# isarandi/metrabs

Measured on AMD Instinct MI355X. Metric: crops/sec (256px, 72 depth bins) at 1/2/4/8 MI355X; MPJPE vs ref, higher is better.
Workload: dtype f32

## Files before the change

### metrabs_amd/backbones.py

```python
import collections
import threading

import torch
import torch.nn.functional as F
from torch import nn


class DepthwiseConv2d(nn.Conv2d):

    use_miopen = False
    _backend_lock = threading.Lock()

    def forward(self, x):
        if x.is_cuda and not DepthwiseConv2d.use_miopen and torch.backends.cudnn.enabled:
            cudnn = torch.backends.cudnn
            with DepthwiseConv2d._backend_lock, cudnn.flags(
                    enabled=False, benchmark=cudnn.benchmark, deterministic=cudnn.deterministic,
                    allow_tf32=cudnn.allow_tf32):
                return super().forward(x)
        return super().forward(x)


class ConvBNAct(nn.Sequential):

# ... 211 lines not shown
        self.b = ConvBNAct(cout, cout, 3, 1, act=None, eps=1e-5)
        self.down = None if stride == 1 and cin == cout else ConvBNAct(cin, cout, 1, stride, act=None, eps=1e-5)

    def forward(self, x):
        idt = x if self.down is None else self.down(x)
        return torch.relu(self.b(self.a(x)) + idt)


def resnet18():
    layers = [ConvBNAct(3, 64, 7, 2, act=nn.ReLU, eps=1e-5), nn.MaxPool2d(3, 2, 1)]
    cin = 64
    for cout, stride in [(64, 1), (128, 2), (256, 2), (512, 2)]:
        layers += [BasicBlock(cin, cout, stride), BasicBlock(cout, cout, 1)]
        cin = cout
    net = nn.Sequential(*layers)
    net.out_channels = 512
    return net


class MBv3Block(nn.Module):
    def __init__(self, cin, k, exp, cout, se, hs, stride):
        super().__init__()
        act = nn.Hardswish if hs else nn.ReLU
        self.residual = stride == 1 and cin == cout
        layers = []
        if exp != cin:
            layers.append(ConvBNAct(cin, exp, 1, 1, act=act))
        layers.append(ConvBNAct(exp, exp, k, stride, groups=exp, act=act))
        if se:
            layers.append(SqueezeExcite(exp, max(8, exp // 4), gate=nn.Hardsigmoid, act=nn.ReLU))
        layers.append(ConvBNAct(exp, cout, 1, 1, act=None))
        self.block = nn.Sequential(*layers)

    def forward(self, x):
        return _block_plus_skip(self.block, x) if self.residual else self.block(x)


def mobilenet_v3_large():
    table = [(3, 16, 16, 0, 0, 1), (3, 64, 24, 0, 0, 2), (3, 72, 24, 0, 0, 1), (5, 72, 40, 1, 0, 2),
             (5, 120, 40, 1, 0, 1), (5, 120, 40, 1, 0, 1), (3, 240, 80, 0, 1, 2), (3, 200, 80, 0, 1, 1),
             (3, 184, 80, 0, 1, 1), (3, 184, 80, 0, 1, 1), (3, 480, 112, 1, 1, 1), (3, 672, 112, 1, 1, 1),
             (5, 672, 160, 1, 1, 2), (5, 960, 160, 1, 1, 1), (5, 960, 160, 1, 1, 1)]
    layers = [Preproc(), ConvBNAct(3, 16, 3, 2, act=nn.Hardswish)]
    cin = 16
    for k, exp, cout, se, hs, s in table:
        layers.append(MBv3Block(cin, k, exp, cout, bool(se), bool(hs), s))
        cin = cout
    layers += [ConvBNAct(cin, 960, 1, 1, act=nn.Hardswish), ConvBNAct(960, 1280, 1, 1, act=nn.Hardswish)]
    net = nn.Sequential(*layers)
    net.out_channels = 1280
    return net


def build_backbone(name):
    name = name.lower()
    if name in ('efficientnetv2-s', 'effnetv2-s', 'effv2s'):
        return efficientnetv2('s')
    if name in ('efficientnetv2-l', 'effnetv2-l', 'effv2l'):
        return efficientnetv2('l')
    if name in ('resnet18', 'resnet-18'):
        return resnet18()
    if name in ('mobilenetv3', 'mobilenetv3-large', 'mobilenet-v3'):
        return mobilenet_v3_large()
    raise ValueError(f'unknown backbone {name}')


_ACT_NAMES = {nn.SiLU: 'silu', nn.ReLU: 'relu', nn.Hardswish: 'hardswish'}


class ConvBiasAct(nn.Module):

    def __init__(self, conv, bias, act):
        super().__init__()
        self.conv = conv
        self.register_buffer('bias', bias.detach().float().contiguous())
        self.act = act
        self.act_name = None if act is None else _ACT_NAMES[type(act)]
        self.emit_mean = False
        self._mean = None
        self._gate = None
        self.last_path = None

    use_k13 = True
    k13_slower = frozenset({(1536, 256, 64)})

    def k13_takes(self, x):
        c = self.conv
        if not (ConvBiasAct.use_k13 and not self.emit_mean and x.is_cuda and c.kernel_size == (1, 1)
                and c.stride == (1, 1) and c.padding == (0, 0) and c.dilation == (1, 1) and c.groups == 1
                and c.bias is None and c.padding_mode == 'zeros'):
            return False
        if torch.is_autocast_enabled('cuda') or (torch.is_grad_enabled() and c.weight.requires_grad):
            return False
        if x.dim() != 4 or (c.in_channels, c.out_channels, x.shape[2] * x.shape[3]) in ConvBiasAct.k13_slower:
            return False
        from . import kernels
        return kernels.conv1x1_supported(x, c.weight)

    def k13_accepts(self, x, residual):
        return self.k13_takes(x) and (residual is None or (residual.dtype == x.dtype and residual.is_contiguous()
                                                           and residual.data_ptr() % 16 == 0))

    use_k13h = True
    k13h_slower = frozenset({(192, 48, 4096), (256, 64, 1024), (1536, 256, 64), (256, 64, 9216), (768, 192, 576),
                             (1152, 224, 576), (1344, 224, 576), (1344, 384, 144), (2304, 384, 144),
                             (2304, 640, 144), (640, 3840, 144), (3840, 640, 144), (640, 1280, 144)})

    def k13h_takes(self, x):
        return self._k13h_takes(x, ConvBiasAct.k13h_slower)

    def _k13h_takes(self, x, slower):
        c = self.conv
        if not (ConvBiasAct.use_k13h and not self.emit_mean and x.is_cuda and x.dtype == c.weight.dtype
                and x.dtype in (torch.float16, torch.bfloat16) and c.kernel_size == (1, 1)
                and c.stride == (1, 1) and c.padding == (0, 0) and c.dilation == (1, 1) and c.groups == 1
                and c.bias is None and c.padding_mode == 'zeros'):
            return False
        if torch.is_autocast_enabled('cuda') or (torch.is_grad_enabled() and c.weight.requires_grad):
            return False
        if x.dim() != 4 or (c.in_channels, c.out_channels, x.shape[2] * x.shape[3]) in slower:
            return False
        from . import kernels
        return kernels.conv1x1_16_supported(x, c.weight)

    deep_projects = False
    deep_config = 'deepk'
    k13h_deep_slower = frozenset({(3840, 640, 144)})

    def k13h_deep_takes(self, x):
        return self.deep_projects and self._k13h_takes(x, ConvBiasAct.k13h_deep_slower)

    def give_gate(self, x, gate):
        self._gate = (x, gate)

    def take_mean_f32(self, x):
        held, self._mean = self._mean, None
        if held is not None and held[0] is x:
            return held[1]
        return None

    def take_mean(self, x):
        m = self.take_mean_f32(x)
        return None if m is None else m.to(x.dtype).view(x.shape[0], x.shape[1], 1, 1)

    def forward(self, x, residual=None, defer_epilogue=False, pre=None):
        if defer_epilogue:
            self.last_path = 'library'
            return self.conv(x)
        if pre is not None:
            from . import kernels
            self._gate, self.last_path = None, 'k13'
            return kernels.conv1x1_bias_act(x, self.conv.weight, self.bias, self.act_name, residual=residual,
                                            in_bias=pre.bias, in_act=pre.act_name)
        held, self._gate = self._gate, None
        gate = held[1] if held is not None and held[0] is x else None
        w16 = self.conv.weight.dtype
        if x.dtype != w16 and w16 in (torch.float16, torch.bfloat16) and not torch.is_autocast_enabled(x.device.type):
            x = x.to(w16)
        skip_ok = residual is None or (residual.dtype == x.dtype and residual.is_contiguous()
                                       and residual.data_ptr() % 16 == 0)
        if skip_ok and self.k13h_deep_takes(x):
            from . import kernels
            self.last_path = 'k13h_deep' if gate is None else 'k13h_deep_gate'
            return kernels.conv1x1_bias_act16(x, self.conv.weight, self.bias, self.act_name, gate=gate,
                                              residual=residual, config=ConvBiasAct.deep_config)
        if skip_ok and self.k13h_takes(x):
            from . import kernels
# ... 359 lines not shown
```

### metrabs_amd/csrc/conv1x1.hip

```cpp
#include <type_traits>

#include "common.h"

namespace mtr {

typedef float f32x16 __attribute__((ext_vector_type(16)));

constexpr int kC1PadX = 32;
constexpr int kC1PadW = 4;

template <int WM, int WN, int FM, int FN, int BK, int ACT, int PRE>
__global__ __launch_bounds__(64 * WM * WN) void conv1x1_kernel(
    const float* __restrict__ x, const float* __restrict__ w, const float* __restrict__ bias,
    const float* __restrict__ in_bias, const float* __restrict__ gate, const float* __restrict__ residual,
    float* __restrict__ y, int M, int K, int HW, int n_total, FastDiv by_hw) {
  constexpr int NT = 64 * WM * WN;
  constexpr int BM = 32 * FM * WM, BN = 32 * FN * WN;
  constexpr int LDX = BN + kC1PadX, LDW = BM + kC1PadW;
  constexpr int XROW4 = BN / 4;
  constexpr int XPASS = NT / XROW4;
  constexpr int XV = (BK + XPASS - 1) / XPASS;
  constexpr int WPASS = NT / (BK / 4);
  constexpr int WV = (BM + WPASS - 1) / WPASS;
  static_assert(NT % XROW4 == 0 && NT % (BK / 4) == 0, "loader mapping");
// ... 180 lines not shown
  auto store_tile = [&](int stage, int kt, auto set) {
    constexpr int P = decltype(set)::value;
    const int k0 = kt * kDkBK;
    const float g = has_gate ? rg[P] : 1.0f;
    const bool x_ok = xcol_ok && k0 + xk < K;
    float* xd = &xs[stage * XS + xk * kDkBN + xp];
    float v0 = rx[P][0], v1 = rx[P][XV - 1];
    if constexpr (PRE >= 0) {
      v0 = settled(activate<PRE>(v0 + rbi[P]));
      if constexpr (XV == 2) v1 = settled(activate<PRE>(v1 + rbi[P]));
    }
    if constexpr (XV == 2) {
      *reinterpret_cast<float2*>(xd) = make_float2(x_ok ? v0 * g : 0.0f, x_ok ? v1 * g : 0.0f);
    } else {
      *xd = x_ok ? v0 * g : 0.0f;
    }
    const bool k_ok = k0 + wk4 * 4 < K;
#pragma unroll
    for (int v = 0; v < 4; ++v) {
      const int row = wr0 + v * (NT / 8);
      const bool ok = k_ok && m0 + row < M;
      float4 u = rw[P][v];
      u.x = ok ? u.x : 0.0f; u.y = ok ? u.y : 0.0f; u.z = ok ? u.z : 0.0f; u.w = ok ? u.w : 0.0f;
      *reinterpret_cast<float4*>(&ws[stage * WS + row * kDkLDW + wk4 * 4]) = u;
    }
  };

  f32x4 acc[2];
#pragma unroll
  for (int f = 0; f < 2; ++f)
#pragma unroll
    for (int r = 0; r < 4; ++r) acc[f][r] = 0.0f;

  const int c = lane & 15, kg = lane >> 4;
  auto multiply = [&](int stage, int kk0) {
    const float* xb_ = &xs[stage * XS + kg * kDkBN + c];
    const float* wb_ = &ws[stage * WS + (wave * 32 + c) * kDkLDW + kg];
#pragma unroll
    for (int kk = kk0; kk < kk0 + kDkBK / 2; kk += 4) {
      const float a = xb_[kk * kDkBN];
      const float b0 = wb_[kk], b1 = wb_[16 * kDkLDW + kk];
      acc[0] = __builtin_amdgcn_mfma_f32_16x16x4f32(a, b0, acc[0], 0, 0, 0);
      acc[1] = __builtin_amdgcn_mfma_f32_16x16x4f32(a, b1, acc[1], 0, 0, 0);
    }
  };

  const int n_tiles = (K + kDkBK - 1) / kDkBK;
  constexpr std::integral_constant<int, 0> ra{};
  constexpr std::integral_constant<int, 1> rb{};
  load_tile(0, ra);
  if (n_tiles > 1) load_tile(1, rb);
  store_tile(0, 0, ra);
  if (n_tiles > 1) store_tile(1, 1, rb);
  if (n_tiles > 2) load_tile(2, ra);
  __syncthreads();
  int stage = 0;
  auto step = [&](int t, auto hold, auto issue, auto guarded) {
    constexpr bool G = decltype(guarded)::value;
    if (!G || t + 3 < n_tiles) load_tile(t + 3, issue);
    multiply(stage, 0);
    __builtin_amdgcn_sched_barrier(0);
    if (!G || t + 2 < n_tiles) store_tile(stage == 0 ? 2 : stage - 1, t + 2, hold);
    __builtin_amdgcn_sched_barrier(0);
    multiply(stage, kDkBK / 2);
    stage = stage == 2 ? 0 : stage + 1;
    __syncthreads();
  };
  int t = 0;
  for (; t + 4 < n_tiles; t += 2) {
    step(t, ra, rb, std::false_type{});
    step(t + 1, rb, ra, std::false_type{});
  }
  for (; t < n_tiles; t += 2) {
    step(t, ra, rb, std::true_type{});
    if (t + 1 < n_tiles) step(t + 1, rb, ra, std::true_type{});
  }

  const int col = n0 + 4 * kg;
  if (col >= n_total) return;
  const unsigned b = fastdiv((unsigned)col, by_hw);
#pragma unroll
  for (int f = 0; f < 2; ++f) {
    const int m = m0 + wave * 32 + f * 16 + c;
    if (m >= M) continue;
    const float bm = bias[m];
    const long long off = ((long long)b * M + m) * HW + (col - (int)b * HW);
    float4 r;
    r.x = activate<ACT>(acc[f][0] + bm);
    r.y = activate<ACT>(acc[f][1] + bm);
    r.z = activate<ACT>(acc[f][2] + bm);
    r.w = activate<ACT>(acc[f][3] + bm);
    if (residual) {
      const float4 q = *reinterpret_cast<const float4*>(residual + off);
      r.x += q.x; r.y += q.y; r.z += q.z; r.w += q.w;
    }
    *reinterpret_cast<float4*>(y + off) = r;
  }
}

constexpr int kStR = 16;
constexpr int kStWaves = 4;
constexpr size_t kStMaxWeight = 64 * 1024;

inline int stream_kpad(int K) { return (K + 2 * kStR - 1) / (2 * kStR) * (2 * kStR); }
inline bool stream_fits(int M, int K) {
  return M <= 96 && (size_t)stream_kpad(K) * ((M + 31) / 32 * 32) * sizeof(float) <= kStMaxWeight;
}

template <int MT, int PRE, bool GATE>
__global__ __launch_bounds__(64 * kStWaves) void conv1x1_stream_kernel(
    const float* __restrict__ x, const float* __restrict__ w, const float* __restrict__ bias,
    const float* __restrict__ in_bias, const float* __restrict__ gate, const float* __restrict__ residual,
    float* __restrict__ y, int M, int K, int HW, int n_total, FastDiv by_hw, int act, int tiles) {
  constexpr int NT = 64 * kStWaves, LDW = 32 * MT;
  extern __shared__ float4 st_lds[];
  const int Kpad = (K + 2 * kStR - 1) / (2 * kStR) * (2 * kStR);
  float* ws = reinterpret_cast<float*>(st_lds);
  float* bs = ws + Kpad * LDW;

  const int tid = threadIdx.x, lane = tid & 63, wave = tid >> 6;
  const int half = lane >> 5, l32 = lane & 31;
  const long long khw = (long long)K * HW;
  const int n_chunks = Kpad / (2 * kStR);
  const int n0 = blockIdx.x * (32 * kStWaves * tiles);

  int col0 = 0;
  bool ok = false;
  const float* xsrc = x;
  const float* gsrc = x;
  auto enter_tile = [&](int tile) {
    col0 = n0 + tile * 32;
    const int col = col0 + l32;
    ok = col < n_total;
    const unsigned b = ok ? fastdiv((unsigned)col, by_hw) : 0u;
    xsrc = x + (long long)b * khw + (long long)half * HW + (ok ? col - (int)b * HW : 0);
    if constexpr (GATE) gsrc = gate + (long long)b * K + half;
  };

  float xa[kStR], xb[kStR], ga[kStR], gb[kStR];
  auto load_chunk = [&](int c, float (&xr)[kStR], float (&gr)[kStR]) {
#pragma unroll
    for (int j = 0; j < kStR; ++j) {
      const int kk = min(c * (2 * kStR) + 2 * j, K - 2);
      xr[j] = xsrc[(long long)kk * HW];
      if constexpr (GATE) gr[j] = gsrc[kk];
    }
  };

  f32x16 acc[MT];
  auto multiply_chunk = [&](int c, const float (&xr)[kStR], const float (&gr)[kStR]) {
#pragma unroll
    for (int j = 0; j < kStR; ++j) {
      const int k = c * (2 * kStR) + 2 * j;
      float v = xr[j];
      if constexpr (PRE >= 0) v = settled(activate<PRE>(v + bs[k + half]));
      if constexpr (GATE) v *= gr[j];
      v = (ok && k < K) ? v : 0.0f;
      const float* wb_ = &ws[(k + half) * LDW + l32];
#pragma unroll
      for (int i = 0; i < MT; ++i) acc[i] = __builtin_amdgcn_mfma_f32_32x32x2f32(v, wb_[i * 32], acc[i], 0, 0, 0);
    }
  };

  enter_tile(wave);
  load_chunk(0, xa, ga);

  for (int e = tid; e < (Kpad / 4) * LDW; e += NT) {
    const int m = e % LDW, k = (e / LDW) * 4;
    float4 t = make_float4(0.0f, 0.0f, 0.0f, 0.0f);
    if (m < M && k < K) t = *reinterpret_cast<const float4*>(w + (long long)m * K + k);
    float* d = &ws[k * LDW + m];
    d[0] = t.x; d[LDW] = t.y; d[2 * LDW] = t.z; d[3 * LDW] = t.w;
  }
  if constexpr (PRE >= 0)
    for (int k = tid; k < Kpad; k += NT) bs[k] = k < K ? in_bias[k] : 0.0f;
  __syncthreads();

  for (int tile = wave;;) {
#pragma unroll
    for (int i = 0; i < MT; ++i)
#pragma unroll
      for (int r = 0; r < 16; ++r) acc[i][r] = 0.0f;
    int c = 0;
    for (; c + 1 < n_chunks; c += 2) {
      load_chunk(c + 1, xb, gb);
      multiply_chunk(c, xa, ga);
      load_chunk(c + 2, xa, ga);
      multiply_chunk(c + 1, xb, gb);
    }
    if (c < n_chunks) multiply_chunk(c, xa, ga);

    auto epilogue = [&](auto act_c) {
      constexpr int ACT = decltype(act_c)::value;
#pragma unroll
      for (int i = 0; i < MT; ++i) {
        const int m = i * 32 + l32;
        if (m >= M) continue;
        const float bm = bias[m];
#pragma unroll
        for (int g = 0; g < 4; ++g) {
          const int col = col0 + 8 * g + 4 * half;
          if (col >= n_total) continue;
          const unsigned b = fastdiv((unsigned)col, by_hw);
          const long long off = ((long long)b * M + m) * HW + (col - (int)b * HW);
          float4 r;
          r.x = activate<ACT>(acc[i][4 * g + 0] + bm);
          r.y = activate<ACT>(acc[i][4 * g + 1] + bm);
          r.z = activate<ACT>(acc[i][4 * g + 2] + bm);
          r.w = activate<ACT>(acc[i][4 * g + 3] + bm);
          if (residual) {
            const float4 q = *reinterpret_cast<const float4*>(residual + off);
            r.x += q.x; r.y += q.y; r.z += q.z; r.w += q.w;
          }
          *reinterpret_cast<float4*>(y + off) = r;
        }
      }
    };
    switch (act) {
      case kActRelu: epilogue(std::integral_constant<int, kActRelu>{}); break;
      case kActSilu: epilogue(std::integral_constant<int, kActSilu>{}); break;
      case kActHardswish: epilogue(std::integral_constant<int, kActHardswish>{}); break;
      default: epilogue(std::integral_constant<int, kActNone>{}); break;
    }

    tile += kStWaves;
    if (tile >= kStWaves * tiles) break;
    enter_tile(tile);
    load_chunk(0, xa, ga);
  }
}

enum Conv1x1Config { kCfgWide = 0, kCfgSquare = 1, kCfgTall = 2, kCfgDeepK = 3, kCfgStream = 4, kCfgCount = 5 };

struct Conv1x1Plan { int cfg, waves_m, bm, bn; };

inline Conv1x1Plan plan_tall(int M) {
  const int w = M <= 160 ? (M + 31) / 32 : 4;
  return {kCfgTall, w, 32 * w, 32};
}
inline Conv1x1Plan plan_deepk(int M) {
  const int w = M <= 128 ? 4 : 8;
  return {kCfgDeepK, w, 32 * w, kDkBN};
}

inline Conv1x1Plan plan_stream(int M, int K, int HW, long long B) {
  if (!stream_fits(M, K)) return plan_tall(M);
  const int t = (B * HW + 127) / 128 >= 2048 ? 2 : 1;
  return {kCfgStream, (M + 31) / 32, (M + 31) / 32 * 32, 32 * kStWaves * t};
}

inline Conv1x1Plan pick_config(int M, int K, int HW, long long B) {
  const long long n_total = B * HW;
  const long long n_tiles128 = (n_total + 127) / 128;
  if (M == 48 && K <= 192 && HW == 4096 && stream_fits(M, K)) return plan_stream(M, K, HW, B);
  if (M <= 160) return plan_tall(M);
  if (M == 256 && K >= 512) return HW <= 64 ? plan_deepk(M) : plan_tall(M);
  if (M >= 1024 && M % 128 == 0 && K <= 256 && n_tiles128 <= 32) return plan_tall(M);
  if (M % 192 == 0 && (M / 192) * n_tiles128 >= 512) return {kCfgWide, 2, 192, 128};
  return {kCfgSquare, 2, 128, 128};
}

inline int plan_for(int M, int K, int HW, long long B, int config, Conv1x1Plan* p) {
  switch (config) {
    case -1: *p = pick_config(M, K, HW, B); return MTR_OK;
    case kCfgWide: *p = {kCfgWide, 2, 192, 128}; return MTR_OK;
    case kCfgSquare: *p = {kCfgSquare, 2, 128, 128}; return MTR_OK;
    case kCfgTall: *p = plan_tall(M); return MTR_OK;
    case kCfgDeepK: *p = plan_deepk(M); return MTR_OK;
    case kCfgStream: *p = plan_stream(M, K, HW, B); return MTR_OK;
    default: return MTR_E_PARAM;
  }
}

template <int WM, int WN, int FM, int FN, int BK, int PRE>
static int launch_conv1x1_pre(const float* x, const float* w, const float* bias, const float* in_bias,
                              const float* gate, const float* residual, float* y, int act, int M, int K, int HW,
                              long long n_total, hipStream_t stream) {
  constexpr int BM = 32 * FM * WM, BN = 32 * FN * WN;
  const long long gx = (n_total + BN - 1) / BN, gy = (M + BM - 1) / BM;
  if (gx > 0x7fffffffLL || gy > 65535) return MTR_E_SHAPE;
  const dim3 grid((unsigned)gx, (unsigned)gy), block(64 * WM * WN);
  const FastDiv by_hw = make_fastdiv((unsigned)HW);
  MTR_CLEAR_STALE();
#define MTR_C1_LAUNCH(ACT)                                                                                      \
  hipLaunchKernelGGL((conv1x1_kernel<WM, WN, FM, FN, BK, ACT, PRE>), grid, block, 0, stream, x, w, bias, in_bias, \
                     gate, residual, y, M, K, HW, (int)n_total, by_hw)
  switch (act) {
    case kActNone: MTR_C1_LAUNCH(kActNone); break;
    case kActRelu: MTR_C1_LAUNCH(kActRelu); break;
    case kActSilu: MTR_C1_LAUNCH(kActSilu); break;
    case kActHardswish: MTR_C1_LAUNCH(kActHardswish); break;
    default: return MTR_E_PARAM;
  }
#undef MTR_C1_LAUNCH
  MTR_CHECK_LAUNCH();
  return MTR_OK;
}

template <int WM, int WN, int FM, int FN, int BK>
static int launch_conv1x1_cfg(const float* x, const float* w, const float* bias, const float* in_bias, int in_act,
                              const float* gate, const float* residual, float* y, int act, int M, int K, int HW,
                              long long n_total, hipStream_t stream) {
#define MTR_C1_PRE(PRE) \
  launch_conv1x1_pre<WM, WN, FM, FN, BK, PRE>(x, w, bias, in_bias, gate, residual, y, act, M, K, HW, n_total, stream)
  switch (in_bias ? in_act : -1) {
    case -1: return MTR_C1_PRE(-1);
    case kActNone: return MTR_C1_PRE(kActNone);
    case kActRelu: return MTR_C1_PRE(kActRelu);
    case kActSilu: return MTR_C1_PRE(kActSilu);
    case kActHardswish: return MTR_C1_PRE(kActHardswish);
    default: return MTR_E_PARAM;
  }
#undef MTR_C1_PRE
}

template <int WAVES, int PRE>
static int launch_conv1x1_deepk_pre(const float* x, const float* w, const float* bias, const float* in_bias,
                                    const float* gate, const float* residual, float* y, int act, int M, int K,
                                    int HW, long long n_total, hipStream_t stream) {
  constexpr int BM = 32 * WAVES;
  constexpr size_t lds = deepk_lds_bytes(WAVES);
  const long long gx = (n_total + kDkBN - 1) / kDkBN, gy = (M + BM - 1) / BM;
  if (gx > 0x7fffffffLL || gy > 65535) return MTR_E_SHAPE;
  const dim3 grid((unsigned)gx, (unsigned)gy), block(64 * WAVES);
  const FastDiv by_hw = make_fastdiv((unsigned)HW);
#define MTR_DK_LAUNCH(ACT)                                                                                 \
  do {                                                                                                     \
    if (lds > 64 * 1024) {                                                                                 \
      const int e = allow_dynamic_lds((const void*)conv1x1_deepk_kernel<WAVES, ACT, PRE>, lds);            \
      if (e != MTR_OK) return e;                                                                           \
    }                                                                                                      \
    MTR_CLEAR_STALE();                                                                                     \
    hipLaunchKernelGGL((conv1x1_deepk_kernel<WAVES, ACT, PRE>), grid, block, lds, stream, x, w, bias,      \
                       in_bias, gate, residual, y, M, K, HW, (int)n_total, by_hw);                         \
  } while (0)
  switch (act) {
    case kActNone: MTR_DK_LAUNCH(kActNone); break;
    case kActRelu: MTR_DK_LAUNCH(kActRelu); break;
    case kActSilu: MTR_DK_LAUNCH(kActSilu); break;
    case kActHardswish: MTR_DK_LAUNCH(kActHardswish); break;
    default: return MTR_E_PARAM;
  }
#undef MTR_DK_LAUNCH
  MTR_CHECK_LAUNCH();
  return MTR_OK;
}

template <int WAVES>
static int launch_conv1x1_deepk(const float* x, const float* w, const float* bias, const float* in_bias,
                                int in_act, const float* gate, const float* residual, float* y, int act, int M,
                                int K, int HW, long long n_total, hipStream_t stream) {
#define MTR_DK_PRE(PRE) \
  launch_conv1x1_deepk_pre<WAVES, PRE>(x, w, bias, in_bias, gate, residual, y, act, M, K, HW, n_total, stream)
  switch (in_bias ? in_act : -1) {
    case -1: return MTR_DK_PRE(-1);
    case kActNone: return MTR_DK_PRE(kActNone);
    case kActRelu: return MTR_DK_PRE(kActRelu);
    case kActSilu: return MTR_DK_PRE(kActSilu);
    case kActHardswish: return MTR_DK_PRE(kActHardswish);
    default: return MTR_E_PARAM;
  }
#undef MTR_DK_PRE
}

template <int MT, int PRE>
static int launch_conv1x1_stream_pre(const float* x, const float* w, const float* bias, const float* in_bias,
                                     const float* gate, const float* residual, float* y, int act, int M, int K,
                                     int HW, long long n_total, int bn, hipStream_t stream) {
  const int kpad = stream_kpad(K);
  const size_t lds = ((size_t)kpad * 32 * MT + (PRE >= 0 ? kpad : 0)) * sizeof(float);
  const long long gx = (n_total + bn - 1) / bn;
  if (gx > 0x7fffffffLL) return MTR_E_SHAPE;
  if (act < kActNone || act > kActHardswish) return MTR_E_PARAM;
  const dim3 grid((unsigned)gx), block(64 * kStWaves);
  const FastDiv by_hw = make_fastdiv((unsigned)HW);
#define MTR_ST_LAUNCH(GATE)                                                                               \
  do {                                                                                                    \
    if (lds > 64 * 1024) {                                                                                \
      const int e = allow_dynamic_lds((const void*)conv1x1_stream_kernel<MT, PRE, GATE>, lds);            \
      if (e != MTR_OK) return e;                                                                          \
    }                                                                                                     \
    MTR_CLEAR_STALE();                                                                                    \
    hipLaunchKernelGGL((conv1x1_stream_kernel<MT, PRE, GATE>), grid, block, lds, stream, x, w, bias,      \
                       in_bias, gate, residual, y, M, K, HW, (int)n_total, by_hw, act,                    \
                       bn / (32 * kStWaves));                                                             \
  } while (0)
  if (gate) MTR_ST_LAUNCH(true); else MTR_ST_LAUNCH(false);
#undef MTR_ST_LAUNCH
  MTR_CHECK_LAUNCH();
  return MTR_OK;
}

template <int MT>
static int launch_conv1x1_stream(const float* x, const float* w, const float* bias, const float* in_bias,
                                 int in_act, const float* gate, const float* residual, float* y, int act, int M,
                                 int K, int HW, long long n_total, int bn, hipStream_t stream) {
#define MTR_ST_PRE(PRE) \
  launch_conv1x1_stream_pre<MT, PRE>(x, w, bias, in_bias, gate, residual, y, act, M, K, HW, n_total, bn, stream)
  switch (in_bias ? in_act : -1) {
    case -1: return MTR_ST_PRE(-1);
    case kActNone: return MTR_ST_PRE(kActNone);
    case kActRelu: return MTR_ST_PRE(kActRelu);
    case kActSilu: return MTR_ST_PRE(kActSilu);
    case kActHardswish: return MTR_ST_PRE(kActHardswish);
    default: return MTR_E_PARAM;
  }
#undef MTR_ST_PRE
}

}

extern "C" int mtr_conv1x1_plan(int M, int K, int HW, long long B, int config, int* plan) {
  if (!plan) return MTR_E_NULL;
  if (B < 0 || M <= 0 || K <= 0 || HW <= 0) return MTR_E_SHAPE;
  mtr::Conv1x1Plan p;
  const int e = mtr::plan_for(M, K, HW, B, config, &p);
  if (e != MTR_OK) return e;
  plan[0] = p.cfg; plan[1] = p.waves_m; plan[2] = p.bm; plan[3] = p.bn;
  return MTR_OK;
}

extern "C" int mtr_conv1x1_bias_act(const void* x, int dtype, const float* weight, const float* bias,
                                    const float* gate, const void* residual, int act, long long B, int M,
                                    int K, int HW, void* y, mtr_stream_t stream) {
  return mtr_conv1x1_bias_act_pre(x, dtype, weight, bias, nullptr, mtr::kActNone, gate, residual, act, B, M, K, HW, y,
                                  stream, -1);
}

extern "C" int mtr_conv1x1_bias_act_opts(const void* x, int dtype, const float* weight, const float* bias,
                                         const float* gate, const void* residual, int act, long long B,
                                         int M, int K, int HW, void* y, mtr_stream_t stream, int config) {
  if (config > mtr::kCfgDeepK) return x && weight && bias && y ? MTR_E_PARAM : MTR_E_NULL;
  return mtr_conv1x1_bias_act_pre(x, dtype, weight, bias, nullptr, mtr::kActNone, gate, residual, act, B, M, K, HW, y,
                                  stream, config);
}

extern "C" int mtr_conv1x1_bias_act_pre(const void* x, int dtype, const float* weight, const float* bias,
                                        const float* in_bias, int in_act, const float* gate, const void* residual,
                                        int act, long long B, int M, int K, int HW, void* y, mtr_stream_t stream,
                                        int config) {
  if (!x || !weight || !bias || !y) return MTR_E_NULL;
  if (dtype != MTR_F32) return MTR_E_DTYPE;
  if (B < 0 || M <= 0 || K <= 0 || HW <= 0) return MTR_E_SHAPE;
  if (HW % 4 || K % 4) return MTR_E_SHAPE;
  if (B * HW > 0x7fffffffLL || (long long)K * HW > 0x7fffffffLL || (long long)M * HW > 0x7fffffffLL)
    return MTR_E_SHAPE;
  if (act < mtr::kActNone || act > mtr::kActHardswish) return MTR_E_PARAM;
  if (in_act < mtr::kActNone || in_act > mtr::kActHardswish) return MTR_E_PARAM;
  if (!in_bias && in_act != mtr::kActNone) return MTR_E_PARAM;
  if (((uintptr_t)x % 16) || ((uintptr_t)weight % 16) || ((uintptr_t)y % 16) || ((uintptr_t)residual % 16) ||
      ((uintptr_t)in_bias % 4))
    return MTR_E_ALIGN;
  if (x == y || (residual && residual == x)) return MTR_E_PARAM;
  if (B == 0) return MTR_OK;
  const float* xf = (const float*)x;
  const float* rf = (const float*)residual;
  float* yf = (float*)y;
  const long long n_total = B * HW;
  hipStream_t s = (hipStream_t)stream;
  mtr::Conv1x1Plan p;
  if (mtr::plan_for(M, K, HW, B, config, &p) != MTR_OK) return MTR_E_PARAM;
#define MTR_C1_ARGS xf, weight, bias, in_bias, in_act, gate, rf, yf, act, M, K, HW, n_total, s
#define MTR_C1_ARGS_ST xf, weight, bias, in_bias, in_act, gate, rf, yf, act, M, K, HW, n_total, p.bn, s
  switch (p.cfg) {
    case mtr::kCfgWide: return mtr::launch_conv1x1_cfg<2, 2, 3, 2, 16>(MTR_C1_ARGS);
    case mtr::kCfgSquare: return mtr::launch_conv1x1_cfg<2, 2, 2, 2, 16>(MTR_C1_ARGS);
    case mtr::kCfgStream:
      switch (p.waves_m) {
        case 1: return mtr::launch_conv1x1_stream<1>(MTR_C1_ARGS_ST);
        case 2: return mtr::launch_conv1x1_stream<2>(MTR_C1_ARGS_ST);
        default: return mtr::launch_conv1x1_stream<3>(MTR_C1_ARGS_ST);
      }
    case mtr::kCfgDeepK:
      switch (p.waves_m) {
        case 4: return mtr::launch_conv1x1_deepk<4>(MTR_C1_ARGS);
        default: return mtr::launch_conv1x1_deepk<8>(MTR_C1_ARGS);
      }
    default:
      switch (p.waves_m) {
        case 1: return mtr::launch_conv1x1_cfg<1, 1, 1, 1, 16>(MTR_C1_ARGS);
        case 2: return mtr::launch_conv1x1_cfg<2, 1, 1, 1, 16>(MTR_C1_ARGS);
        case 3: return mtr::launch_conv1x1_cfg<3, 1, 1, 1, 16>(MTR_C1_ARGS);
        case 4: return mtr::launch_conv1x1_cfg<4, 1, 1, 1, 32>(MTR_C1_ARGS);
        default: return mtr::launch_conv1x1_cfg<5, 1, 1, 1, 16>(MTR_C1_ARGS);
      }
  }
#undef MTR_C1_ARGS
#undef MTR_C1_ARGS_ST
}
```

### metrabs_amd/kernels.py

```python
import ctypes

import torch

from metrabs_amd import _lib
from metrabs_amd._lib import check, current_stream_ptr, dtype_code, require_cuda


def _ptr(t):
    return ctypes.c_void_p(t.data_ptr()) if t is not None else ctypes.c_void_p(0)


def softargmax_decode(logits, n_points, cfg, out=None, nhwc_staging=0):
    require_cuda(logits)
    lib = _lib.load()
    nhwc = _is_channels_last(logits)
    if not nhwc:
        logits = logits.contiguous()
    B, n_out, H, W = logits.shape
    J = int(n_points)
    D = n_out // J - 1
    if n_out != J * (1 + D) or D != cfg.depth:
        raise ValueError(f'logits have {n_out} channels, expected J*(1+depth) = {J * (1 + cfg.depth)}')
    if out is None:
        c2d = torch.empty(B, J, 2, device=logits.device, dtype=torch.float32)
# ... 504 lines not shown
def depthwise3x3_blocks_plan(dtype, H, W):
    import ctypes
    cols = ctypes.c_int(0)
    rc = _lib.load().mtr_depthwise3x3_blocks_supported(dtype_code(dtype), int(H), int(W), 1, 1, 1, 1, 1,
                                                       ctypes.addressof(cols))
    return cols.value if rc == 0 else None


def depthwise3x3_blocks_bias_act(x, weight, bias, act, want_mean=False, block_cols=None):
    require_cuda(x, weight, bias)
    if not x.is_contiguous():
        raise ValueError('depthwise3x3_blocks_bias_act needs an NCHW-contiguous tensor')
    if weight.numel() != x.shape[1] * 9:
        raise ValueError(f'depthwise3x3_blocks_bias_act needs a [C, 3, 3] weight, got {tuple(weight.shape)}')
    if block_cols not in (None, 4, 8):
        raise ValueError(f'depthwise3x3_blocks_bias_act: block_cols must be None, 4 or 8, got {block_cols}')
    B, C, H, W = x.shape
    y = torch.empty(B, C, H, W, device=x.device, dtype=x.dtype)
    mean = torch.empty(B, C, device=x.device, dtype=torch.float32) if want_mean else None
    check(_lib.load().mtr_depthwise3x3_blocks_bias_act_opts(
        _ptr(x), dtype_code(x.dtype), _ptr(weight.contiguous().float()), _ptr(bias.contiguous().float()),
        ACT_CODES[act], B, C, H, W, _ptr(y), None if mean is None else _ptr(mean),
        current_stream_ptr(x.device), int(block_cols or 0)), 'mtr_depthwise3x3_blocks_bias_act_opts')
    return (y, mean) if want_mean else y


def depthwise5x5_supported(H, W, pad):
    pl, pr, pt, pb = (pad,) * 4 if isinstance(pad, int) else tuple(int(p) for p in pad)
    return H + pt + pb <= 112 and W + pl + pr <= 112


def depthwise5x5_bias_act(x, weight, bias, act, stride, pad, want_mean=False):
    require_cuda(x, weight, bias)
    if not x.is_contiguous():
        raise ValueError('depthwise5x5_bias_act needs an NCHW-contiguous tensor')
    if weight.numel() != x.shape[1] * 25:
        raise ValueError(f'depthwise5x5_bias_act needs a [C, 5, 5] weight, got {tuple(weight.shape)}')
    B, C, H, W = x.shape
    pl, pr, pt, pb = (pad,) * 4 if isinstance(pad, int) else tuple(int(p) for p in pad)
    OH, OW = (H + pt + pb - 5) // stride + 1, (W + pl + pr - 5) // stride + 1
    y = torch.empty(B, C, max(OH, 0), max(OW, 0), device=x.device, dtype=x.dtype)
    mean = torch.empty(B, C, device=x.device, dtype=torch.float32) if want_mean else None
    check(_lib.load().mtr_depthwise5x5_bias_act_padded(
        _ptr(x), dtype_code(x.dtype), _ptr(weight.contiguous().float()), _ptr(bias.contiguous().float()),
        ACT_CODES[act], B, C, H, W, int(stride), pt, pl, pb, pr, _ptr(y), None if mean is None else _ptr(mean),
        current_stream_ptr(x.device)), 'mtr_depthwise5x5_bias_act_padded')
    return (y, mean) if want_mean else y



SE_GATE_CODES = {'sigmoid': 0, 'hardsigmoid': 1}


def se_gate(mean, w1, b1, w2, b2, act, gate_fn, out=None, w2t=None, config=-1):
    require_cuda(mean, w1, b1, w2, b2, w2t)
    B, C = mean.shape[0], mean.shape[1]
    S = w1.shape[0]
    w1, w2 = w1.reshape(S, -1), w2.reshape(C, -1)
    if mean.dtype != torch.float32 or mean.numel() != B * C or w1.shape[1] != C or w2.shape[1] != S:
        raise ValueError('se_gate: mean [B, C] f32, w1 [S, C], w2 [C, S]')
    if w2t is not None:
        if w2t.shape != (S, C) or w2t.dtype != torch.float32 or not w2t.is_contiguous():
            raise ValueError('se_gate: w2t must be [S, C] f32, contiguous')
        w2 = w2t
    tensors = [t.contiguous().float() for t in (mean, w1, b1, w2, b2)]
    if out is None:
        out = torch.empty(B, C, device=mean.device, dtype=torch.float32)
    check(_lib.load().mtr_se_gate_opts(*(_ptr(t) for t in tensors), ACT_CODES[act], SE_GATE_CODES[gate_fn], B, C,
                                       S, _ptr(out), current_stream_ptr(mean.device),
                                       0 if w2t is None else 1, int(config)), 'mtr_se_gate_opts')
    return out



def conv1x1_supported(x, weight):
    if x.dim() != 4 or x.dtype != torch.float32 or weight.dtype != torch.float32 or not x.is_contiguous():
        return False
    K, HW = x.shape[1], x.shape[2] * x.shape[3]
    return (weight.numel() == weight.shape[0] * K and HW % 4 == 0 and K % 4 == 0
            and x.data_ptr() % 16 == 0 and weight.data_ptr() % 16 == 0
            and x.shape[0] * HW < 2 ** 31 and K * HW < 2 ** 31 and weight.shape[0] * HW < 2 ** 31)


CONV1X1_CONFIGS = {'auto': -1, 'wide': 0, 'square': 1, 'tall': 2, 'deepk': 3, 'stream': 4}


def conv1x1_plan(M, K, HW, B, config='auto'):
    import ctypes
    plan = (ctypes.c_int * 4)()
    check(_lib.load().mtr_conv1x1_plan(M, K, HW, B, CONV1X1_CONFIGS[config], ctypes.addressof(plan)),
          'mtr_conv1x1_plan')
    names = {v: k for k, v in CONV1X1_CONFIGS.items()}
    return names[plan[0]], plan[1], plan[2], plan[3]


def conv1x1_bias_act(x, w, bias, act, gate=None, residual=None, out=None, config='auto', in_bias=None, in_act=None):
    require_cuda(x, w, bias, gate, residual, in_bias)
    B, K, H, W = x.shape
    M = w.shape[0]
    w = w.reshape(M, -1)
    if w.shape[1] != K:
        raise ValueError(f'conv1x1_bias_act: weight has {w.shape[1]} input channels, x has {K}')
    if gate is not None and (gate.dtype != torch.float32 or gate.numel() != B * K):
        raise ValueError('conv1x1_bias_act: gate must be [B, Cin] f32')
    if in_bias is None and in_act is not None:
        raise ValueError('conv1x1_bias_act: in_act needs in_bias')
    if in_bias is not None and (in_bias.dtype != torch.float32 or in_bias.numel() != K):
        raise ValueError('conv1x1_bias_act: in_bias must be [Cin] f32')
    if residual is not None and (residual.shape != (B, M, H, W) or residual.dtype != x.dtype
                                 or not residual.is_contiguous()):
        raise ValueError('conv1x1_bias_act: residual must be [B, Cout, H, W] like the output, contiguous')
    if out is None:
        out = torch.empty(B, M, H, W, device=x.device, dtype=x.dtype)
    elif out.shape != (B, M, H, W) or out.dtype != x.dtype or not out.is_contiguous():
        raise ValueError('conv1x1_bias_act: out must be [B, Cout, H, W] like the output, contiguous')
    check(_lib.load().mtr_conv1x1_bias_act_pre(
        _ptr(x), dtype_code(x.dtype), _ptr(w.contiguous()), _ptr(bias.contiguous().float()),
        None if in_bias is None else _ptr(in_bias.contiguous()), ACT_CODES[in_act],
        None if gate is None else _ptr(gate.contiguous()), None if residual is None else _ptr(residual),
        ACT_CODES[act], B, M, K, H * W, _ptr(out), current_stream_ptr(x.device), CONV1X1_CONFIGS[config]),
        'mtr_conv1x1_bias_act_pre')
    return out



def conv1x1_16_supported(x, weight):
    if x.dim() != 4 or x.dtype not in (torch.float16, torch.bfloat16) or weight.dtype != x.dtype \
            or not x.is_contiguous() or not weight.is_contiguous():
        return False
    K, HW = x.shape[1], x.shape[2] * x.shape[3]
    return (weight.numel() == weight.shape[0] * K and HW % 8 == 0 and K % 8 == 0
            and x.data_ptr() % 16 == 0 and weight.data_ptr() % 16 == 0
            and x.shape[0] * HW < 2 ** 31 and K * HW < 2 ** 31 and weight.shape[0] * HW < 2 ** 31)


CONV1X1_16_CONFIGS = {'auto': -1, 'tall': 0, 'square': 1, 'deepk': 2}


def conv1x1_16_plan(M, K, HW, B, config='auto'):
    import ctypes
    plan = (ctypes.c_int * 4)()
    check(_lib.load().mtr_conv1x1_plan16(M, K, HW, B, CONV1X1_16_CONFIGS[config], ctypes.addressof(plan)),
          'mtr_conv1x1_plan16')
    names = {v: k for k, v in CONV1X1_16_CONFIGS.items()}
    return names[plan[0]], plan[1], plan[2], plan[3]


def conv1x1_bias_act16(x, w, bias, act, gate=None, residual=None, out=None, config='auto'):
    require_cuda(x, w, bias, gate, residual)
    code = CONV1X1_16_CONFIGS[config]
    B, K, H, W = x.shape
    M = w.shape[0]
    w = w.reshape(M, -1)
    if w.shape[1] != K:
        raise ValueError(f'conv1x1_bias_act16: weight has {w.shape[1]} input channels, x has {K}')
    if w.dtype != x.dtype:
        raise ValueError(f'conv1x1_bias_act16: weight is {w.dtype}, x is {x.dtype}')
    if gate is not None and (gate.dtype != torch.float32 or gate.numel() != B * K):
        raise ValueError('conv1x1_bias_act16: gate must be [B, Cin] f32')
    if residual is not None and (residual.shape != (B, M, H, W) or residual.dtype != x.dtype
                                 or not residual.is_contiguous()):
        raise ValueError('conv1x1_bias_act16: residual must be [B, Cout, H, W] like the output, contiguous')
    if out is None:
        out = torch.empty(B, M, H, W, device=x.device, dtype=x.dtype)
    elif out.shape != (B, M, H, W) or out.dtype != x.dtype or not out.is_contiguous():
        raise ValueError('conv1x1_bias_act16: out must be [B, Cout, H, W] like the output, contiguous')
    args = (_ptr(x), dtype_code(x.dtype), _ptr(w.contiguous()), _ptr(bias.contiguous().float()),
# ... 159 lines not shown
```

Baseline: 8985.

## Add 64x64 three-stage pipelined conv1x1 kernel for selected shape classes

Adds a new 1x1-conv GEMM kernel with 64x64 tiles, BK=32 and a three-stage LDS ring. Global-to-register prefetch is split around two half-K MFMA passes so loads overlap compute, and the x tile uses an XOR swizzle. The planner sends a hard-coded list of (M,K,HW) shape classes to it, and the Python-side exclusion of the (1536,256,64) shape from the custom path is removed so that layer now uses the new kernel too. The gain depends on the table of shapes matching the network, and other shapes stay on the old configs.

```diff
diff --git a/metrabs_amd/backbones.py b/metrabs_amd/backbones.py
--- a/metrabs_amd/backbones.py
+++ b/metrabs_amd/backbones.py
@@ -317,7 +317,7 @@
         self.last_path = None
 
     use_k13 = True
-    k13_slower = frozenset({(1536, 256, 64)})
+    k13_slower = frozenset()
 
     def k13_takes(self, x):
         c = self.conv
diff --git a/metrabs_amd/csrc/conv1x1.hip b/metrabs_amd/csrc/conv1x1.hip
--- a/metrabs_amd/csrc/conv1x1.hip
+++ b/metrabs_amd/csrc/conv1x1.hip
@@ -286,6 +286,160 @@
 #pragma unroll
   for (int f = 0; f < 2; ++f) {
     const int m = m0 + wave * 32 + f * 16 + c;
+    if (m >= M) continue;
+    const float bm = bias[m];
+    const long long off = ((long long)b * M + m) * HW + (col - (int)b * HW);
+    float4 r;
+    r.x = activate<ACT>(acc[f][0] + bm);
+    r.y = activate<ACT>(acc[f][1] + bm);
+    r.z = activate<ACT>(acc[f][2] + bm);
+    r.w = activate<ACT>(acc[f][3] + bm);
+    if (residual) {
+      const float4 q = *reinterpret_cast<const float4*>(residual + off);
+      r.x += q.x; r.y += q.y; r.z += q.z; r.w += q.w;
+    }
+    *reinterpret_cast<float4*>(y + off) = r;
+  }
+}
+
+constexpr int kD6BM = 64, kD6BN = 64, kD6BK = 32, kD6Stages = 3, kD6Waves = 8;
+constexpr int kD6LDW = kD6BK + 2;
+
+template <int ACT, int PRE>
+__global__ __launch_bounds__(64 * kD6Waves) void conv1x1_deep64_kernel(
+    const float* __restrict__ x, const float* __restrict__ w, const float* __restrict__ bias,
+    const float* __restrict__ in_bias, const float* __restrict__ gate, const float* __restrict__ residual,
+    float* __restrict__ y, int M, int K, int HW, int n_total, FastDiv by_hw) {
+  constexpr int NT = 64 * kD6Waves, BM = kD6BM, BN = kD6BN, BK = kD6BK, LDW = kD6LDW;
+  constexpr int XS = BK * BN, WS = BM * LDW;
+  static_assert(BK * (BN / 4) == NT && BM * (BK / 4) == NT, "loader mappings: one 16-byte group of x and of W each");
+  __shared__ __attribute__((aligned(16))) float d6_lds[kD6Stages * (XS + WS)];
+  float* xs = d6_lds;
+  float* ws = d6_lds + kD6Stages * XS;
+
+  const int tid = threadIdx.x, lane = tid & 63, wave = tid >> 6;
+  const int wm = wave & 1, wn = wave >> 1;
+  const int m0 = blockIdx.y * BM, n0 = blockIdx.x * BN;
+  const long long khw = (long long)K * HW;
+
+  const int xn4 = tid & 15, xk = tid >> 4;
+  const int xcol = n0 + 4 * xn4;
+  const bool xcol_ok = xcol < n_total;
+  const unsigned xb = xcol_ok ? fastdiv((unsigned)xcol, by_hw) : 0u;
+  const float* xsrc = xcol_ok ? x + (long long)xb * khw + (xcol - (int)xb * HW) : x;
+  const bool has_gate = gate != nullptr;
+  const float* gsrc = has_gate ? gate + (long long)xb * K : x;
+  const int xdst = xk * BN + ((4 * xn4) ^ ((xk & 1) << 4));
+  const int wk4 = tid & 7, wr = tid >> 3;
+  const float* wsrc = w + (long long)min(m0 + wr, M - 1) * K;
+  const bool wrow_ok = m0 + wr < M;
+  const int wdst = wr * LDW + 4 * wk4;
+  const float* xcur = xsrc + (long long)(3 * BK + xk) * HW;
+  const float* gcur = gsrc + 3 * BK + xk;
+  const float* bcur = PRE >= 0 ? in_bias + 3 * BK + xk : nullptr;
+  const float* wcur = wsrc + 3 * BK + 4 * wk4;
+  const long long xadv = (long long)BK * HW;
+
+  const float4 zero = make_float4(0.0f, 0.0f, 0.0f, 0.0f);
+  float4 rx[2] = {zero, zero}, rw[2] = {zero, zero};
+  float rg[2] = {1.0f, 1.0f}, rbi[2] = {0.0f, 0.0f};
+  auto load_tile = [&](int kt, auto set) {
+    constexpr int P = decltype(set)::value;
+    const int k0 = kt * BK;
+    const int kx = min(k0 + xk, K - 1);
+    rx[P] = *reinterpret_cast<const float4*>(xsrc + (long long)kx * HW);
+    rg[P] = gsrc[kx];
+    if constexpr (PRE >= 0) rbi[P] = in_bias[kx];
+    rw[P] = *reinterpret_cast<const float4*>(wsrc + min(k0 + 4 * wk4, K - 4));
+  };
+  auto load_next_whole_tile = [&](auto set) {
+    constexpr int P = decltype(set)::value;
+    rx[P] = *reinterpret_cast<const float4*>(xcur);
+    rg[P] = *gcur;
+    if constexpr (PRE >= 0) rbi[P] = *bcur;
+    rw[P] = *reinterpret_cast<const float4*>(wcur);
+    xcur += xadv; gcur += BK; wcur += BK;
+    if constexpr (PRE >= 0) bcur += BK;
+  };
+  auto store_tile = [&](int stage, int kt, auto set) {
+    constexpr int P = decltype(set)::value;
+    const int k0 = kt * BK;
+    const float g = has_gate ? rg[P] : 1.0f;
+    const bool x_ok = xcol_ok && k0 + xk < K;
+    float4 v = rx[P];
+    if constexpr (PRE >= 0) {
+      const float bi = rbi[P];
+      v.x = settled(activate<PRE>(v.x + bi)); v.y = settled(activate<PRE>(v.y + bi));
+      v.z = settled(activate<PRE>(v.z + bi)); v.w = settled(activate<PRE>(v.w + bi));
+    }
+    v.x = x_ok ? v.x * g : 0.0f; v.y = x_ok ? v.y * g : 0.0f; v.z = x_ok ? v.z * g : 0.0f; v.w = x_ok ? v.w * g : 0.0f;
+    *reinterpret_cast<float4*>(&xs[stage * XS + xdst]) = v;
+    const bool ok = wrow_ok && k0 + 4 * wk4 < K;
+    const float4 u = rw[P];
+    float* wd = &ws[stage * WS + wdst];
+    *reinterpret_cast<float2*>(wd) = make_float2(ok ? u.x : 0.0f, ok ? u.y : 0.0f);
+    *reinterpret_cast<float2*>(wd + 2) = make_float2(ok ? u.z : 0.0f, ok ? u.w : 0.0f);
+  };
+
+  f32x4 acc[2];
+#pragma unroll
+  for (int f = 0; f < 2; ++f)
+#pragma unroll
+    for (int r = 0; r < 4; ++r) acc[f][r] = 0.0f;
+
+  const int c = lane & 15, kg = lane >> 4;
+  const int xfrag = kg * BN + ((wn * 16 + c) ^ ((kg & 1) << 4));
+  const int wfrag = (wm * 32 + c) * LDW + kg;
+  auto multiply = [&](int stage, int kk0) {
+    const float* xb_ = &xs[stage * XS + xfrag];
+    const float* wb_ = &ws[stage * WS + wfrag];
+#pragma unroll
+    for (int kk = kk0; kk < kk0 + BK / 2; kk += 4) {
+      const float a = xb_[kk * BN];
+      const float b0 = wb_[kk], b1 = wb_[16 * LDW + kk];
+      acc[0] = __builtin_amdgcn_mfma_f32_16x16x4f32(a, b0, acc[0], 0, 0, 0);
+      acc[1] = __builtin_amdgcn_mfma_f32_16x16x4f32(a, b1, acc[1], 0, 0, 0);
+    }
+  };
+
+  const int n_tiles = (K + BK - 1) / BK, n_whole = K / BK;
+  constexpr std::integral_constant<int, 0> ra{};
+  constexpr std::integral_constant<int, 1> rb{};
+  load_tile(0, ra);
+  if (n_tiles > 1) load_tile(1, rb);
+  store_tile(0, 0, ra);
+  if (n_tiles > 1) store_tile(1, 1, rb);
+  if (n_tiles > 2) load_tile(2, ra);
+  __syncthreads();
+  int stage = 0;
+  auto step = [&](int t, auto hold, auto issue, auto guarded) {
+    constexpr bool G = decltype(guarded)::value;
+    if constexpr (!G) load_next_whole_tile(issue);
+    else if (t + 3 < n_tiles) load_tile(t + 3, issue);
+    multiply(stage, 0);
+    __builtin_amdgcn_sched_barrier(0);
+    if (!G || t + 2 < n_tiles) store_tile(stage == 0 ? 2 : stage - 1, t + 2, hold);
+    __builtin_amdgcn_sched_barrier(0);
+    multiply(stage, BK / 2);
+    stage = stage == 2 ? 0 : stage + 1;
+    __syncthreads();
+  };
+  int t = 0;
+  for (; t + 4 < n_whole; t += 2) {
+    step(t, ra, rb, std::false_type{});
+    step(t + 1, rb, ra, std::false_type{});
+  }
+  for (; t < n_tiles; t += 2) {
+    step(t, ra, rb, std::true_type{});
+    if (t + 1 < n_tiles) step(t + 1, rb, ra, std::true_type{});
+  }
+
+  const int col = n0 + wn * 16 + 4 * kg;
+  if (col >= n_total) return;
+  const unsigned b = fastdiv((unsigned)col, by_hw);
+#pragma unroll
+  for (int f = 0; f < 2; ++f) {
+    const int m = m0 + wm * 32 + f * 16 + c;
     if (m >= M) continue;
     const float bm = bias[m];
     const long long off = ((long long)b * M + m) * HW + (col - (int)b * HW);
@@ -434,7 +588,9 @@
   }
 }
 
-enum Conv1x1Config { kCfgWide = 0, kCfgSquare = 1, kCfgTall = 2, kCfgDeepK = 3, kCfgStream = 4, kCfgCount = 5 };
+enum Conv1x1Config {
+  kCfgWide = 0, kCfgSquare = 1, kCfgTall = 2, kCfgDeepK = 3, kCfgStream = 4, kCfgDeep64 = 5, kCfgCount = 6
+};
 
 struct Conv1x1Plan { int cfg, waves_m, bm, bn; };
 
@@ -446,6 +602,8 @@
   const int w = M <= 128 ? 4 : 8;
   return {kCfgDeepK, w, 32 * w, kDkBN};
 }
+
+inline Conv1x1Plan plan_deep64() { return {kCfgDeep64, 2, kD6BM, kD6BN}; }
 
 inline Conv1x1Plan plan_stream(int M, int K, int HW, long long B) {
   if (!stream_fits(M, K)) return plan_tall(M);
@@ -453,9 +611,21 @@
   return {kCfgStream, (M + 31) / 32, (M + 31) / 32 * 32, 32 * kStWaves * t};
 }
 
+inline bool deep64_measured_faster(int M, int K, int HW) {
+  static const int classes[][3] = {
+      {256, 64, 1024}, {128, 256, 256}, {512, 128, 256}, {128, 512, 256},
+      {160, 768, 256}, {960, 160, 256}, {160, 960, 256},
+      {256, 960, 64},  {1536, 256, 64}, {256, 1536, 64}, {1280, 256, 64},
+  };
+  for (const auto& c : classes)
+    if (c[0] == M && c[1] == K && c[2] == HW) return true;
+  return false;
+}
+
 inline Conv1x1Plan pick_config(int M, int K, int HW, long long B) {
   const long long n_total = B * HW;
   const long long n_tiles128 = (n_total + 127) / 128;
+  if (deep64_measured_faster(M, K, HW)) return plan_deep64();
   if (M == 48 && K <= 192 && HW == 4096 && stream_fits(M, K)) return plan_stream(M, K, HW, B);
   if (M <= 160) return plan_tall(M);
   if (M == 256 && K >= 512) return HW <= 64 ? plan_deepk(M) : plan_tall(M);
@@ -472,6 +642,7 @@
     case kCfgTall: *p = plan_tall(M); return MTR_OK;
     case kCfgDeepK: *p = plan_deepk(M); return MTR_OK;
     case kCfgStream: *p = plan_stream(M, K, HW, B); return MTR_OK;
+    case kCfgDeep64: *p = plan_deep64(); return MTR_OK;
     default: return MTR_E_PARAM;
   }
 }
@@ -565,6 +736,46 @@
     default: return MTR_E_PARAM;
   }
 #undef MTR_DK_PRE
+}
+
+template <int PRE>
+static int launch_conv1x1_deep64_pre(const float* x, const float* w, const float* bias, const float* in_bias,
+                                     const float* gate, const float* residual, float* y, int act, int M, int K,
+                                     int HW, long long n_total, hipStream_t stream) {
+  const long long gx = (n_total + kD6BN - 1) / kD6BN, gy = (M + kD6BM - 1) / kD6BM;
+  if (gx > 0x7fffffffLL || gy > 65535) return MTR_E_SHAPE;
+  const dim3 grid((unsigned)gx, (unsigned)gy), block(64 * kD6Waves);
+  const FastDiv by_hw = make_fastdiv((unsigned)HW);
+  MTR_CLEAR_STALE();
+#define MTR_D6_LAUNCH(ACT)                                                                                    \
+  hipLaunchKernelGGL((conv1x1_deep64_kernel<ACT, PRE>), grid, block, 0, stream, x, w, bias, in_bias, gate,    \
+                     residual, y, M, K, HW, (int)n_total, by_hw)
+  switch (act) {
+    case kActNone: MTR_D6_LAUNCH(kActNone); break;
+    case kActRelu: MTR_D6_LAUNCH(kActRelu); break;
+    case kActSilu: MTR_D6_LAUNCH(kActSilu); break;
+    case kActHardswish: MTR_D6_LAUNCH(kActHardswish); break;
+    default: return MTR_E_PARAM;
+  }
+#undef MTR_D6_LAUNCH
+  MTR_CHECK_LAUNCH();
+  return MTR_OK;
+}
+
+static int launch_conv1x1_deep64(const float* x, const float* w, const float* bias, const float* in_bias,
+                                 int in_act, const float* gate, const float* residual, float* y, int act, int M,
+                                 int K, int HW, long long n_total, hipStream_t stream) {
+#define MTR_D6_PRE(PRE) \
+  launch_conv1x1_deep64_pre<PRE>(x, w, bias, in_bias, gate, residual, y, act, M, K, HW, n_total, stream)
+  switch (in_bias ? in_act : -1) {
+    case -1: return MTR_D6_PRE(-1);
+    case kActNone: return MTR_D6_PRE(kActNone);
+    case kActRelu: return MTR_D6_PRE(kActRelu);
+    case kActSilu: return MTR_D6_PRE(kActSilu);
+    case kActHardswish: return MTR_D6_PRE(kActHardswish);
+    default: return MTR_E_PARAM;
+  }
+#undef MTR_D6_PRE
 }
 
 template <int MT, int PRE>
@@ -675,6 +886,7 @@
         case 2: return mtr::launch_conv1x1_stream<2>(MTR_C1_ARGS_ST);
         default: return mtr::launch_conv1x1_stream<3>(MTR_C1_ARGS_ST);
       }
+    case mtr::kCfgDeep64: return mtr::launch_conv1x1_deep64(MTR_C1_ARGS);
     case mtr::kCfgDeepK:
       switch (p.waves_m) {
         case 4: return mtr::launch_conv1x1_deepk<4>(MTR_C1_ARGS);
diff --git a/metrabs_amd/kernels.py b/metrabs_amd/kernels.py
--- a/metrabs_amd/kernels.py
+++ b/metrabs_amd/kernels.py
@@ -610,7 +610,7 @@
             and x.shape[0] * HW < 2 ** 31 and K * HW < 2 ** 31 and weight.shape[0] * HW < 2 ** 31)
 
 
-CONV1X1_CONFIGS = {'auto': -1, 'wide': 0, 'square': 1, 'tall': 2, 'deepk': 3, 'stream': 4}
+CONV1X1_CONFIGS = {'auto': -1, 'wide': 0, 'square': 1, 'tall': 2, 'deepk': 3, 'stream': 4, 'deep64': 5}
 
 
 def conv1x1_plan(M, K, HW, B, config='auto'):
```

Measured after the change: 9486, median of 6. +5.6%, better.
